# hugocornellier/face_detection_tflite

Hardware: NVIDIA B200
Metric: images/sec BlazeFace detect (pre+infer+NMS) (higher is better)
Workload: dtype f32

## Files before the change

face_detection_tflite_b200/csrc/engine.cu:

```cuda
#include "engine.h"

#include <algorithm>
#include <cstdio>
#include <cstdlib>

namespace fdt {

Engine::~Engine() {
  if (d_blob_) cudaFree(d_blob_);
  for (TailLayerD* p : d_tail_) if (p) cudaFree(p);
  for (TailBlk* p : d_blks_) if (p) cudaFree(p);
}

bool Engine::init(const uint8_t* tflite, size_t len, int fuse_level, std::string* err, bool use_tc) {
  if (!model_.parse(tflite, len, err)) return false;
  if (!plan_.build(model_, fuse_level, err, use_tc)) return false;
  size_t bytes = plan_.blob.size() * sizeof(float) + 64;
  if (cudaMalloc(&d_blob_, bytes) != cudaSuccess) { *err = "cudaMalloc(weights) failed"; return false; }
  cudaMemset(d_blob_, 0, bytes);
  if (cudaMemcpy(d_blob_, plan_.blob.data(), plan_.blob.size() * sizeof(float), cudaMemcpyHostToDevice) != cudaSuccess) {
    *err = "weight upload failed";
    return false;
  }
  d_tail_.assign(plan_.steps.size(), nullptr);
// ... 200 lines not shown
        p.in_floats = st.in_stage_floats;
        if (!launch_block_ws(p, B, ctx.cap, s)) { failed_ = true; fprintf(stderr, "fdt: k_block_ws could not be launched for step '%s'\n", st.name.c_str()); }
        break;
      }
      case kStepTailWs: {
        TailP p;
        TV iv = view(ctx, st.in);
        p.in = iv.p; p.in_istride = iv.istride; p.H = iv.H; p.W = iv.W; p.CinS = iv.Cs;
        p.blob = blob; p.layers = d_tail_[&st - plan_.steps.data()]; p.nlayers = (int)st.tail.size();
        p.nbuf = st.tail_nbuf;
        for (int k = 0; k < kTailMaxBufs; ++k) { p.buf_off[k] = st.tail_buf_off[k]; p.buf_ks[k] = st.tail_buf_ks[k]; }
        p.act_floats = st.tail_act_floats; p.in_bytes = st.tail_in_bytes;
        p.generic = 0;
        for (const TailLayerD& L : st.tail)
          if (L.kind >= 2 || L.act == 2 || L.w_parts != 1 || L.wscale != 1.f || L.rbuf != L.src || (L.kind != 1 && L.o1 >= 0)) p.generic = 1;
        p.blks = nullptr; p.nblks = 0; p.bias_floats = 0; p.in_px = iv.H * iv.W;
        for (int k = 0; k < 2; ++k) { p.rsrc[k] = nullptr; p.rs_istride[k] = 0; p.rs_cs[k] = p.rs_w[k] = p.rs_c[k] = 0; }
        if (st.tail_wide) {
          p.generic = 2;
          p.blks = d_blks_[&st - plan_.steps.data()]; p.nblks = (int)st.tail_blks.size(); p.bias_floats = st.tail_bias_floats;
          for (size_t k = 0; k < st.tail_rsrc.size() && k < 2; ++k) {
            TV rv = view(ctx, st.tail_rsrc[k]);
            p.rsrc[k] = rv.p; p.rs_istride[k] = rv.istride; p.rs_cs[k] = rv.Cs; p.rs_w[k] = rv.W; p.rs_c[k] = rv.C;
          }
        }
        p.last_a_layer = st.tail_last_a; p.wbuf_bytes = st.tail_wbuf; p.wdepth = st.tail_wdepth; p.tbuf_bytes = st.tail_tbuf; p.smem_bytes = st.smem;
        for (int k = 0; k < 4; ++k) { p.outs[k] = nullptr; p.out_istride[k] = 0; p.out_pix[k] = 0; }
        for (size_t k = 0; k < st.tail_outs.size(); ++k) {
          TV ov = view(ctx, st.tail_outs[k]);
          p.outs[k] = ov.p; p.out_istride[k] = ov.istride; p.out_pix[k] = ov.Cs;
        }
        if (!launch_tail_ws(p, B, ctx.cap, s)) { failed_ = true; fprintf(stderr, "fdt: k_tail_ws could not be launched for step '%s'\n", st.name.c_str()); }
        break;
      }
      case kStepFcTc: {
        FcP p;
        TV iv = view(ctx, st.in);
        p.in = iv.p; p.in_istride = iv.istride;
        p.out = out.p; p.out_istride = out.istride;
        p.w = blob + st.w; p.bias = blob + st.bias;
        p.K = st.K; p.K16 = st.K8; p.N = st.Cout; p.w_parts = st.w_parts; p.tile_bytes = st.ts_rec_bytes; p.wscale = (float)st.out_scale;
        if (!launch_fc_tc(p, B, s)) { failed_ = true; fprintf(stderr, "fdt: k_fc_tc could not be launched for step '%s'\n", st.name.c_str()); }
        break;
      }
      case kStepBlockTs: {
        BlockTsP p;
        TV iv = view(ctx, st.in);
        p.in = iv.p; p.in_istride = iv.istride; p.H = iv.H; p.W = iv.W; p.CinS = iv.Cs;
        p.out = out.p; p.out_istride = out.istride; p.OH = out.H; p.OW = out.W; p.CoutS = out.Cs;
        p.rec = blob + st.ts_rec; p.bias = blob + st.ts_bias; p.rec_bytes = st.ts_rec_bytes;
        p.Cin = iv.C; p.K16 = st.ts_k16; p.Npad = st.ts_npad; p.KS = st.ts_ks;
        p.stride = st.dws; p.res = st.ts_res; p.relu = st.ts_relu;
        p.wide = (out.Cs % 8 == 0 && out.istride % 8 == 0 && ((size_t)out.p % 32 == 0)) ? 1 : 0;
        p.ns = st.ts_ns; p.stage_bytes = st.ts_stage_bytes; p.smem_bytes = st.smem;
        {
          const float* hdw = plan_.blob.data() + st.ts_rec + (size_t)st.ts_npad * st.ts_k16 / 2;
          for (int q = 0; q < 16; ++q)
            for (int k = 0; k < 10; ++k)
              for (int c = 0; c < 4; ++c) p.dw[(q * 10 + k) * 4 + c] = 4 * q + c < st.ts_k16 ? hdw[k * st.ts_k16 + 4 * q + c] : 0.f;
        }
        if (!launch_block_ts(p, B, ctx.cap, s)) { failed_ = true; fprintf(stderr, "fdt: k_block_ts could not be launched for step '%s'\n", st.name.c_str()); }
        break;
      }
      case kStepAdd: case kStepAct: case kStepPadC: {
        EltP p;
        p.a = view(ctx, st.in);
        p.b = st.in2 >= 0 ? view(ctx, st.in2) : p.a;
        p.out = out;
        p.alpha = st.alpha >= 0 ? blob + st.alpha : nullptr;
        p.act = st.act;
        if (st.kind == kStepAdd) launch_add(p, B, s);
        else if (st.kind == kStepAct) launch_act(p, B, s);
        else launch_padc(p, B, s);
        break;
      }
      case kStepMaxPool: {
        PoolP p;
        p.in = view(ctx, st.in); p.out = out;
        p.fh = st.fh; p.fw = st.fw; p.sh = st.sh; p.sw = st.sw; p.pt = st.pt; p.pl = st.pl;
        launch_maxpool(p, B, s);
        break;
      }
      case kStepResize: {
        ResizeP p;
        p.in = view(ctx, st.in); p.out = out; p.align_corners = st.align; p.half_pixel = st.half;
        p.has_add = st.in2 >= 0 ? 1 : 0; p.act = st.act;
        p.add = st.in2 >= 0 ? view(ctx, st.in2) : p.in;
        launch_resize_bilinear(p, B, s);
        break;
      }
    }
    ++launches;
  }
  if (evs) cudaEventRecord(evs[launches], s);
  return launches;
}

}
```

face_detection_tflite_b200/csrc/fdt_api.cu:

```cuda
#include <cuda_runtime.h>

#include <algorithm>
#include <cmath>
#include <cstdio>
#include <cstdlib>
#include <cstring>
#include <mutex>
#include <string>
#include <thread>
#include <vector>

#include "../../include/fdt_api.h"
#include "engine.h"
#include "jpeg_host.h"
#include "fdt_math.h"
#include "kernels.h"
#include "tile_walk.h"

using namespace fdt;

static_assert(sizeof(fdt_face) == 160, "fdt_face wire layout (bindings rely on it)");
static_assert(sizeof(fdt_config) == 48, "fdt_config layout");

namespace {
// ... 1533 lines not shown
  std::lock_guard<std::mutex> g(h->mu);
  const int S = (int)h->det.plan().steps.size();
  if (out_launches) *out_launches = S + 2;
  FrameLayout lay;
  const char* msg = nullptr;
  if (!d_frames || n <= 0 || n > h->chunk || width <= 0 || height <= 0 || repeats <= 0 ||
      frame_layout(mat_type, width, height, row_stride, &lay, &msg) != FDT_OK)
    return fail(h, FDT_ERR_BAD_ARG, "bad profile arguments");
  if (!out_ms || capacity < S + 2) return fail(h, FDT_ERR_SIZE_MISMATCH, "out_ms too small");
  cudaSetDevice(h->cfg.device);
  if (!ensure_results(h, n)) return FDT_ERR_CUDA;
  const LbTables* tb = get_tables(h, width, height);
  if (!tb) return fail(h, FDT_ERR_CUDA, "letterbox table upload failed");
  std::vector<cudaEvent_t> ev(S + 3);
  for (auto& e : ev) cudaEventCreate(&e);
  std::vector<double> acc(S + 2, 0.0);
  Slot& sl = h->slots[0];
  cudaStream_t s = sl.stream;
  const int S_w = h->det.in_w(), S_h = h->det.in_h();
  for (int r = 0; r < repeats; ++r) {
    cudaEventRecord(ev[0], s);
    if (lay.yuv) {
      LetterboxYuvP lb;
      fill_letterbox_yuv(lb, tb, lay, d_frames, lay.frame_bytes, false, d_frames + lay.c_off, lay.frame_bytes, false, row_stride,
                         width, height, sl.d_lb, S_w, S_h);
      launch_letterbox_yuv(lb, n, s);
    } else {
      LetterboxP lb;
      fill_letterbox(lb, tb, d_frames, lay.frame_bytes, row_stride, lay.channels, width, height, sl.d_lb, S_w, S_h, false);
      launch_letterbox(lb, n, s);
    }
    h->det.run(sl.det_ctx, sl.d_lb, n, s, ev.data() + 1);
    DecodeP d;
    fill_decode(d, h, sl, tb, width, height);
    d.faces = h->d_faces; d.counts = h->d_counts;
    launch_decode_nms(d, n, s);
    cudaEventRecord(ev[S + 2], s);
    if (!cuda_ok(h, cudaStreamSynchronize(s), "profile")) { for (auto& e : ev) cudaEventDestroy(e); return FDT_ERR_CUDA; }
    for (int i = 0; i < S + 2; ++i) {
      float ms = 0;
      cudaEventElapsedTime(&ms, ev[i], ev[i + 1]);
      acc[i] += ms;
    }
  }
  for (int i = 0; i < S + 2; ++i) out_ms[i] = (float)(acc[i] / repeats);
  for (auto& e : ev) cudaEventDestroy(e);
  return FDT_OK;
}

static const char* kKernelNames[] = {"k_normalize", "k_naive_conv", "k_gemm_conv", "k_dwpw", "k_add", "k_act", "k_padc", "k_maxpool",
                                     "k_resize_bilinear", "k_stem", "k_block_ws", "k_stem_ws", "k_tail_ws", "k_fc_tc", "k_block_ts"};

static void step_info(const Plan& p, const PStep& st, int in_w, int in_h, std::string* kname, std::string* tname, double* macs, double* bytes) {
  *kname = kKernelNames[st.kind]; *tname = st.name; *macs = st.macs;
  const PTensor& o = p.tensors[st.out];
  double b = (double)o.H * o.W * o.C * 4;
  if (st.out2 >= 0) { const PTensor& o2 = p.tensors[st.out2]; b += (double)o2.H * o2.W * o2.C * 4; }
  if (st.in_u8) b += (double)in_w * in_h * 4;
  else if (st.in >= 0) { const PTensor& i = p.tensors[st.in]; b += (double)i.H * i.W * i.C * 4; }
  if (st.in2 >= 0 && st.in2 != st.in) { const PTensor& r = p.tensors[st.in2]; b += (double)r.H * r.W * r.C * 4; }
  for (int extra : st.extra_out) { const PTensor& e = p.tensors[extra]; b += (double)e.H * e.W * e.C * 4; }
  *bytes = b;
}

int32_t fdt_get_step_info(fdt_handle* h, int32_t launch, char* kernel, char* tensor, int32_t str_cap, double* macs_per_image,
                          double* bytes_per_image) {
  if (!h || !h->ready) return fail(h, FDT_ERR_NOT_READY, "detector is not initialised");
  h = primary(h);
  const Plan& p = h->det.plan();
  const int S = (int)p.steps.size();
  if (launch < 0 || launch > S + 1) return fail(h, FDT_ERR_BAD_ARG, "launch index out of range");
  std::string kname, tname;
  double macs = 0, bytes = 0;
  if (launch == 0) {
    kname = "k_letterbox"; tname = "letterboxed_u8";
    bytes = 0;
  } else if (launch == S + 1) {
    kname = "k_decode_nms"; tname = "faces";
    bytes = (double)h->num_anchors * 17 * 4;
  } else {
    step_info(p, p.steps[launch - 1], h->det.in_w(), h->det.in_h(), &kname, &tname, &macs, &bytes);
  }
  if (kernel && str_cap > 0) { std::snprintf(kernel, str_cap, "%s", kname.c_str()); }
  if (tensor && str_cap > 0) { std::snprintf(tensor, str_cap, "%s", tname.c_str()); }
  if (macs_per_image) *macs_per_image = macs;
  if (bytes_per_image) *bytes_per_image = bytes;
  return FDT_OK;
}

int32_t fdt_profile_net(fdt_handle* h, int32_t which, int32_t n, int32_t repeats, float* out_ms, int32_t capacity, int32_t* out_steps) {
  if (!h || !h->ready) return fail(h, FDT_ERR_NOT_READY, "detector is not initialised");
  h = primary(h);
  std::lock_guard<std::mutex> g(h->mu);
  if (which != 1 && which != 2) return fail(h, FDT_ERR_BAD_ARG, "which: 1 mesh, 2 iris");
  if ((which == 1 && !h->has_mesh) || (which == 2 && !h->has_iris)) return fail(h, FDT_ERR_NOT_READY, "model not loaded");
  const Engine& e = which == 1 ? h->mesh : h->iris;
  const int S = (int)e.plan().steps.size();
  if (out_steps) *out_steps = S;
  const int have = which == 1 ? h->last_mesh_faces : 2 * h->last_iris_faces;
  if (n <= 0 || n > have) n = have;
  if (out_steps) out_steps[0] = S;
  if (n <= 0 || repeats <= 0) return fail(h, FDT_ERR_BAD_ARG, "the last call left no crops in the stage buffers");
  if (!out_ms || capacity < S) return fail(h, FDT_ERR_SIZE_MISMATCH, "out_ms too small");
  cudaSetDevice(h->cfg.device);
  Slot& sl = h->slots[which == 1 ? h->last_mesh_slot : h->last_iris_slot];
  cudaStream_t s = sl.stream;
  std::vector<cudaEvent_t> ev(S + 1);
// ... 124 lines not shown
```

face_detection_tflite_b200/csrc/kernels.h:

```cpp
#pragma once
#include <cuda_runtime.h>
#include <algorithm>
#include <cstdint>

#include "../../include/fdt_api.h"
#include "tail_layer.h"

namespace fdt {

enum { kActNone = 0, kActRelu = 1, kActPrelu = 2 };

struct FastDiv {
  unsigned mul = 0, shr = 0, d = 1;
  FastDiv() {}
  explicit FastDiv(int div) {
    d = div < 1 ? 1u : (unsigned)div;
    unsigned l = 0;
    while ((1ull << l) < d) ++l;
    shr = l;
    mul = (unsigned)(((1ull << 32) * ((1ull << l) - d)) / d + 1);
  }
#ifdef __CUDACC__
  __device__ __forceinline__ int div(int n) const { return (int)((__umulhi(mul, (unsigned)n) + (unsigned)n) >> shr); }
  __device__ __forceinline__ void divmod(int n, int& q, int& r) const { q = div(n); r = n - q * (int)d; }
// ... 104 lines not shown
  size_t smem_bytes;
};
void launch_dwpw(const DwPwP& p, int B, cudaStream_t s, int max_ctas);

struct DwPwTcP {
  const float* in; long long in_istride; int H, W, Cin, CinS;
  int has_dw, s, dpt, dpl, OH, OW;
  const float* dww;
  const float* dwb;
  int K8, KS;
  float* out; long long out_istride; int Cout, CoutS, vec_store;
  const float* wB;
  const float* bias; const float* alpha;
  int act, Npad, tmem_cols, a_rows, RS;
  int in_floats, n_chunks, n_items;
  int nr, KSr, res_stage_floats;
  int deint, plane_floats, PW;
  int w_parts;
  int nbuf;
  int ns, na, nd, nt;
  int no, KSo, out_stage_floats;
  float* out2; long long out2_istride; int Cs2, c1, c2;
  long long* trace;
  const float* res; long long res_istride; int res_H, res_W, res_C, res_Cs, res_pool, res_mode, res_lim;
  int TH, TW, G, IH, IW, tilesX, tilesY;
  FastDiv fd_Q8, fd_IW, fd_IH, fd_TW, fd_thw, fd_tpg, fd_tilesX, fd_nstrips, fd_nslots;
  size_t smem_bytes;
};
bool launch_block_ws(const DwPwTcP& p, int B, int cap, cudaStream_t s);

struct StemWsP {
  const uint8_t* in8;
  int H, W, OH, OW, kw, pt, pl;
  float* out; long long out_istride; int Cout, CoutS, vec_store;
  const float* wB;
  const float* bias; const float* alpha;
  int act, Npad, K8, tmem_cols, w_parts;
  float out_scale;
  size_t smem_bytes;
};
bool launch_stem_ws(const StemWsP& p, int B, int cap, cudaStream_t s);

struct BlockTsP {
  const float* in; long long in_istride; int H, W, CinS;
  float* out; long long out_istride; int OH, OW, CoutS;
  const float* rec;
  const float* bias;
  int rec_bytes;
  int Cin, K16, Npad, KS;
  int stride;
  int res;
  int relu, wide;
  int ns, stage_bytes;
  size_t smem_bytes;
  alignas(16) float dw[10 * 64];
};
size_t ts_smem_bytes(int rec_bytes, int Npad, int ns, int stage_bytes);
bool launch_block_ts(const BlockTsP& p, int B, int cap, cudaStream_t s);

struct TailP {
  const float* in; long long in_istride; int H, W, CinS;
  const float* blob;
  const TailLayerD* layers;
  int nlayers;
  int nbuf;
  int buf_off[kTailMaxBufs];
  int buf_ks[kTailMaxBufs];
  int act_floats;
  int in_bytes;
  int last_a_layer;
  int wbuf_bytes, wdepth;
  int tbuf_bytes;
  int generic;
  const TailBlk* blks; int nblks; int bias_floats; int in_px;
  const float* rsrc[2]; long long rs_istride[2]; int rs_cs[2], rs_w[2], rs_c[2];
  float* outs[4]; long long out_istride[4]; int out_pix[4];
  size_t smem_bytes;
};
size_t tail_smem_bytes(int act_floats, int wbuf_bytes, int wdepth, int tbuf_bytes);
size_t wide_smem_bytes(int act_floats, int wbuf_bytes, int wdepth, int tbuf_bytes, int bias_floats);
bool launch_tail_ws(const TailP& p, int B, int cap, cudaStream_t s);

struct FcP {
  const float* in; long long in_istride;
  float* out; long long out_istride;
  const float* w;
  const float* bias;
  int K, K16, N, w_parts, tile_bytes;
  float wscale;
};
bool launch_fc_tc(const FcP& p, int B, cudaStream_t s);

struct JpegIdctP {
  const int16_t* coef;
  const uint16_t* q;
  int bw, bh;
  uint8_t* plane; int pitch;
};
struct JpegColorP {
  const uint8_t* py; const uint8_t* pcb; const uint8_t* pcr;
  int pitch_y, pitch_c;
  int W, H, ncomp;
  int cdw, cdh, hs, vs;
  int orientation;
  uint8_t* out; int out_w;
};
// ... 59 lines not shown
```

face_detection_tflite_b200/csrc/kernels_ts.cu:

```cuda
#include <cuda.h>
#include <cuda_fp16.h>

#include <algorithm>
#include <cstdio>
#include <map>
#include <mutex>
#include <tuple>
#include <type_traits>

#include "kernels.h"
#include "tile_walk.h"

namespace fdt {
namespace {

constexpr int kC = 12;
constexpr int kThreads = (kC + 2) * 32;
constexpr uint32_t kLBO = 128;

__device__ __forceinline__ uint32_t smem_u32(const void* p) { return (uint32_t)__cvta_generic_to_shared(p); }
__device__ __forceinline__ void mbar_init(uint32_t bar, uint32_t count) { asm volatile("mbarrier.init.shared::cta.b64 [%0], %1;" ::"r"(bar), "r"(count)); }
__device__ __forceinline__ void mbar_arrive(uint32_t bar) { asm volatile("mbarrier.arrive.shared::cta.b64 _, [%0];" ::"r"(bar) : "memory"); }
__device__ __forceinline__ void mbar_expect_tx(uint32_t bar, uint32_t bytes) {
  asm volatile("mbarrier.arrive.expect_tx.shared::cta.b64 _, [%0], %1;" ::"r"(bar), "r"(bytes) : "memory");
// ... 245 lines not shown
        if (lane == 0) mbar_arrive(in_empty + 8u * (uint32_t)stage);
      }
      at_prev = at; stage_prev = stage;
      tile_advance(at, step, tiles_x, tiles_y);
      if (++stage == NS) { stage = 0; in_phase ^= 1u; }
    }
    if (n_my > 0) epilogue(n_my - 1, stage_prev, at_prev.b, at_prev.ty, at_prev.tx);
  } else if (warp == kC) {
    if (lane == 0) {
      const TileStep step = tile_step((int)gridDim.x, tpi, tiles_x);
      TileAt at = tile_at((int)blockIdx.x, tpi, tiles_x);
      int stage = 0;
      uint32_t empty_phase = 1;
      for (int i = 0; i < n_my; ++i) {
        const int b = at.b, ty = at.ty, tx = at.tx;
        if (i >= NS) mbar_wait_idle(in_empty + 8u * (uint32_t)stage, empty_phase);
        const uint32_t bar = in_full + 8u * (uint32_t)stage;
        mbar_expect_tx(bar, (uint32_t)((S == 1 ? 18 * 18 : 2 * 17 * 17) * KS) * 4u);
        const int ix0 = S == 1 ? tx * TW - 1 : tx * TW * 2, iy0 = S == 1 ? ty * TH - 1 : ty * TH * 2;
        asm volatile("cp.async.bulk.tensor.4d.shared::cluster.global.mbarrier::complete_tx::bytes [%0], [%1, {%2, %3, %4, %5}], [%6];"
                     ::"r"(ring_a + (uint32_t)stage * stage_b), "l"(&tmap), "r"(0), "r"(ix0), "r"(iy0), "r"(b), "r"(bar) : "memory");
        if (S == 2)
          asm volatile("cp.async.bulk.tensor.4d.shared::cluster.global.mbarrier::complete_tx::bytes [%0], [%1, {%2, %3, %4, %5}], [%6];"
                       ::"r"(ring_a + (uint32_t)stage * stage_b + plane_b), "l"(&tmap), "r"(0), "r"(ix0 + 1), "r"(iy0), "r"(b), "r"(bar) : "memory");
        tile_advance(at, step, tiles_x, tiles_y);
        if (++stage == NS) { stage = 0; empty_phase ^= 1u; }
      }
    }
    __syncwarp();
  } else {
    if (lane == 0) {
      const uint32_t idesc = (1u << 4) | ((uint32_t)(p.Npad >> 3) << 17) | ((128u >> 4) << 24);
      const uint32_t sbo = (uint32_t)(p.K16 >> 3) * 128u;
      const uint32_t b_hi = ((sbo >> 4) & 0x3FFFu) | (1u << 14);
      const uint32_t b_lo0 = ((smem_u32(sRec) & 0x3FFFFu) >> 4) | ((kLBO >> 4) << 16);
      const int ksteps = p.K16 >> 4;
      for (int i = 0; i < n_my; ++i) {
        const int slot = i & 1;
        mbar_wait_idle(a_full + 8u * (uint32_t)slot, (uint32_t)((i >> 1) & 1));
        asm volatile("tcgen05.fence::after_thread_sync;" ::: "memory");
#pragma unroll
        for (int t = 0; t < NT; ++t) {
          const uint32_t dcol = tmem_base + col_d(slot, t), acol = tmem_base + col_a(slot, t);
          uint32_t acc = 0u;
#pragma unroll 1
          for (int part = 0; part < 2; ++part)
#pragma unroll 1
            for (int ks = 0; ks < ksteps; ++ks) {
              mma_ts_f16(dcol, acol + 32u * (uint32_t)part + 8u * (uint32_t)ks, b_lo0 + 16u * (uint32_t)ks, b_hi, idesc, acc);
              acc = 1u;
            }
        }
        asm volatile("tcgen05.commit.cta_group::1.mbarrier::arrive::one.shared::cluster.b64 [%0];" ::"r"(d_full + 8u * (uint32_t)slot) : "memory");
      }
    }
    __syncwarp();
  }
  asm volatile("tcgen05.fence::before_thread_sync;" ::: "memory");
  __syncthreads();
  if (warp == kC + 1) {
    asm volatile("tcgen05.fence::after_thread_sync;" ::: "memory");
    asm volatile("tcgen05.dealloc.cta_group::1.sync.aligned.b32 %0, %1;" ::"r"(tmem_base), "r"(512u));
  }
}

typedef CUresult (*EncodeTiledFn)(CUtensorMap*, CUtensorMapDataType, cuuint32_t, void*, const cuuint64_t*, const cuuint64_t*,
                                  const cuuint32_t*, const cuuint32_t*, CUtensorMapInterleave, CUtensorMapSwizzle,
                                  CUtensorMapL2promotion, CUtensorMapFloatOOBfill);

EncodeTiledFn encode_fn() {
  static EncodeTiledFn fn = [] {
    void* f = nullptr;
    cudaDriverEntryPointQueryResult q;
    if (cudaGetDriverEntryPoint("cuTensorMapEncodeTiled", &f, cudaEnableDefault, &q) != cudaSuccess || q != cudaDriverEntryPointSuccess) f = nullptr;
    return (EncodeTiledFn)f;
  }();
  return fn;
}

bool ts_tensor_map(const BlockTsP& p, int cap, CUtensorMap* out) {
  typedef std::tuple<const void*, int, int, int, int, int, int, long long> Key;
  static std::mutex mu;
  static std::map<Key, CUtensorMap> cache;
  Key key(p.in, cap, p.H, p.W, p.CinS, p.KS, p.stride, p.in_istride);
  std::lock_guard<std::mutex> g(mu);
  auto it = cache.find(key);
  if (it != cache.end()) { *out = it->second; return true; }
  EncodeTiledFn enc = encode_fn();
  if (!enc) return false;
  cuuint64_t gdim[4] = {(cuuint64_t)p.CinS, (cuuint64_t)p.W, (cuuint64_t)p.H, (cuuint64_t)cap};
  cuuint64_t gstr[3] = {(cuuint64_t)p.CinS * 4, (cuuint64_t)p.W * p.CinS * 4, (cuuint64_t)p.in_istride * 4};
  cuuint32_t box[4] = {(cuuint32_t)p.KS, p.stride == 1 ? 18u : 33u, p.stride == 1 ? 18u : 17u, 1u};
  cuuint32_t estr[4] = {1, p.stride == 1 ? 1u : 2u, 1, 1};
  CUtensorMap tm;
  CUresult r = enc(&tm, CU_TENSOR_MAP_DATA_TYPE_FLOAT32, 4, const_cast<float*>(p.in), gdim, gstr, box, estr,
                   CU_TENSOR_MAP_INTERLEAVE_NONE, CU_TENSOR_MAP_SWIZZLE_NONE, CU_TENSOR_MAP_L2_PROMOTION_L2_128B,
                   CU_TENSOR_MAP_FLOAT_OOB_FILL_NONE);
  if (r != CUDA_SUCCESS) return false;
  if (cache.size() > 256) cache.clear();
  cache[key] = tm;
  *out = tm;
  return true;
}

template <int S, int KSC>
bool launch_ts(const CUtensorMap& tm, const BlockTsP& p, int B, cudaStream_t s) {
  static std::mutex mu;
  static std::map<int, size_t> cur;
  int dev = 0, sms = 148;
  cudaGetDevice(&dev);
  cudaDeviceGetAttribute(&sms, cudaDevAttrMultiProcessorCount, dev);
  {
    std::lock_guard<std::mutex> g(mu);
    size_t& c = cur[dev];
    if (p.smem_bytes > c) {
      if (cudaFuncSetAttribute(k_block_ts<S, KSC>, cudaFuncAttributeMaxDynamicSharedMemorySize, (int)p.smem_bytes) != cudaSuccess) return false;
      c = p.smem_bytes;
    }
  }
  const int ntiles = B * (p.OW / 16) * (p.OH / (S == 1 ? 16 : 8));
  const int grid = std::max(1, std::min(ntiles, sms));
  k_block_ts<S, KSC><<<grid, kThreads, p.smem_bytes, s>>>(tm, p, B);
  return true;
}

}

size_t ts_smem_bytes(int rec_bytes, int Npad, int ns, int stage_bytes) {
  return (size_t)rec_bytes + (size_t)Npad * 4 + 32 * 8 + 128 + (size_t)ns * stage_bytes + 128;
}

bool launch_block_ts(const BlockTsP& p, int B, int cap, cudaStream_t s) {
  if (B <= 0) return true;
  CUtensorMap tm;
  if (!ts_tensor_map(p, cap, &tm)) return false;
  if (p.stride == 1) {
    switch (p.KS) {
      case 28: return launch_ts<1, 28>(tm, p, B, s);
      case 36: return launch_ts<1, 36>(tm, p, B, s);
      case 44: return launch_ts<1, 44>(tm, p, B, s);
      case 52: return launch_ts<1, 52>(tm, p, B, s);
      default: return launch_ts<1, 0>(tm, p, B, s);
    }
  }
  switch (p.KS) {
    case 28: return launch_ts<2, 28>(tm, p, B, s);
    case 36: return launch_ts<2, 36>(tm, p, B, s);
    case 44: return launch_ts<2, 44>(tm, p, B, s);
    case 52: return launch_ts<2, 52>(tm, p, B, s);
    default: return launch_ts<2, 0>(tm, p, B, s);
  }
}

}
```

face_detection_tflite_b200/csrc/plan.cpp:

```cpp
#include "plan.h"

#include <algorithm>
#include <cmath>
#include <cstdio>
#include <cstdlib>
#include <cstring>
#include <cstdint>

namespace fdt {
namespace {

constexpr size_t kSmemLimit = 200 * 1024;
constexpr int kActNone = 0, kActRelu = 1, kActPrelu = 2;

inline int ru(int v, int m) { return (v + m - 1) / m * m; }
inline int smem_stride(int KP) { return KP + (((KP / 4) % 2 == 0) ? 4 : 0); }

void same_pad(int in, int k, int s, int* before) {
  int out = (in + s - 1) / s;
  int total = (out - 1) * s + k - in;
  if (total < 0) total = 0;
  *before = total / 2;
}

// ... 376 lines not shown
    }
    if (st.has_dw) {
      const TfOp& dw = m.ops[absorbed[0]];
      std::vector<float> dwv, dbv;
      if (!m.const_f32(dw.in[1], &dwv) || !m.const_f32(dw.in[2], &dbv)) return fail("depthwise weights are not constant");
      const int kp = tc ? fs.K8 : st.KP;
      std::vector<float> dk((size_t)9 * kp, 0.f);
      for (int t = 0; t < 9; ++t)
        for (int c = 0; c < Cin; ++c) dk[(size_t)t * kp + c] = dwv[(size_t)t * Cin + c];
      F->st.dww = push(dk, dk.size());
      F->st.dwb = push(dbv, kp);
    }
    F->st.macs = (double)OH * OW * ((double)Cin * st.Cout + (st.has_dw ? 9.0 * Cin : 0.0));
    if (tc && F->st.kind == kStepBlockWs) plan_ts(&F->st, st_in, OH, OW, alpha_tf >= 0);
    return true;
  }

  void plan_ts(PStep* st, const TfTensor& in, int OH, int OW, bool prelu) {
    static const int want = [] { const char* e = std::getenv("FDT_TS"); return e ? std::atoi(e) : 1; }();
    if (!want || !st->has_dw || st->c2 > 0 || st->w_parts != 1 || prelu) return;
    if (st->act != kActRelu && st->act != kActNone) return;
    const int Cin = in.dim(3), K16 = ru(Cin, 16), Npad = ru(st->Cout, 16);
    if (K16 > 64 || Npad > 64) return;
    if (st->dws == 1 ? (OH % 16 || OW % 16 || st->dpt != 1 || st->dpl != 1)
                     : (OH % 8 || OW % 16 || st->dpt != 0 || st->dpl != 0 || in.dim(1) != 2 * OH || in.dim(2) != 2 * OW)) return;
    int res = 0;
    if (st->res_mode != 0) {
      if (st->res_mode != 1) return;
      res = st->res_pool ? 2 : 1;
      if ((res == 2) != (st->dws == 2)) return;
    }
    const size_t SBO8 = (size_t)(st->K8 / 4) * 128, SBO16 = (size_t)(K16 / 8) * 128;
    std::vector<uint16_t> wh((size_t)Npad * K16, 0);
    for (int n = 0; n < st->Cout; ++n)
      for (int k = 0; k < Cin; ++k) {
        const float v = P.blob[(size_t)st->w + ((size_t)(n >> 3) * SBO8 + (size_t)(k >> 2) * 128 + (size_t)(n & 7) * 16 + (size_t)(k & 3) * 4) / 4];
        const uint16_t hbits = f32_to_f16(v);
        if (f16_to_f32(hbits) != v) return;
        wh[((size_t)(n >> 3) * SBO16 + (size_t)(k >> 3) * 128 + (size_t)(n & 7) * 16 + (size_t)(k & 7) * 2) / 2] = hbits;
      }
    std::vector<float> rec(wh.size() / 2 + (size_t)10 * K16, 0.f);
    std::memcpy(rec.data(), wh.data(), wh.size() * 2);
    float* dw = rec.data() + wh.size() / 2;
    for (int k = 0; k < 9; ++k)
      for (int c = 0; c < Cin; ++c) dw[(size_t)k * K16 + c] = P.blob[(size_t)st->dww + (size_t)k * st->K8 + c];
    for (int c = 0; c < Cin; ++c) dw[(size_t)9 * K16 + c] = P.blob[(size_t)st->dwb + c];
    std::vector<float> bias((size_t)Npad, 0.f);
    for (int n = 0; n < st->Cout; ++n) bias[n] = P.blob[(size_t)st->bias + n];
    const int KS = odd_quads(ru(Cin, 4));
    const int stage_bytes = st->dws == 1 ? (18 * 18 * KS * 4 + 127) / 128 * 128 : 2 * ((17 * 17 * KS * 4 + 127) / 128 * 128);
    const size_t head = rec.size() * 4 + (size_t)Npad * 4 + 32 * 8 + 256;
    int ns = (int)(((size_t)220 * 1024 - head) / stage_bytes);
    if (ns < 2) return;
    if (ns > 4) ns = 4;
    st->ts_rec = push(rec, rec.size());
    st->ts_bias = push(bias, bias.size());
    st->ts_rec_bytes = (int)(rec.size() * 4);
    st->ts_k16 = K16; st->ts_npad = Npad; st->ts_ks = KS; st->ts_ns = ns; st->ts_stage_bytes = stage_bytes;
    st->ts_res = res; st->ts_relu = st->act == kActRelu ? 1 : 0;
    st->TH = st->dws == 1 ? 16 : 8; st->TW = 16; st->G = 1;
    st->smem = head + (size_t)ns * stage_bytes;
    st->kind = kStepBlockTs;
  }

  static void split_w(float v, int parts, float* hi, float* lo) {
    if (parts == 1) { *hi = v; return; }
    uint32_t u;
    std::memcpy(&u, &v, 4);
    u &= 0xFFFFE000u;
    float h;
    std::memcpy(&h, &u, 4);
    *hi = h;
    *lo = v - h;
  }

  static bool tf32_exact(const std::vector<float>& w) {
    for (float v : w) {
      uint32_t u;
      std::memcpy(&u, &v, 4);
      if (u & 0x1FFFu) return false;
    }
    return true;
  }

  bool plan_tc(PStep* st, int Cin, int OH, int OW, int w_parts) {
    PStep s = *st;
    s.w_parts = w_parts;
    s.K8 = ru(Cin, 8);
    s.Npad = ru(s.Cout, 16);
    if (s.Npad > 128 || s.K8 > 256) return false;
    s.KS = s.K8 + (((s.K8 / 4) % 2 == 0) ? 4 : 0);
    s.tmem_cols = 32;
    while (s.tmem_cols < s.Npad) s.tmem_cols *= 2;
    for (int Pn = 128; Pn >= 32; Pn /= 2) {
      const size_t cap = (size_t)220 * 1024;
      s.TM = 1; s.NPG = Pn;
      int bestTH = 0, bestTW = 0, bestG = 1;
      double best = -1;
      if (OH * OW <= Pn && OW <= 30) {
        bestTH = OH; bestTW = OW; bestG = std::min(63, Pn / (OH * OW));
      } else {
        for (int TW = std::min(std::min(OW, Pn), 30); TW >= 1; --TW) {
          int TH = std::min(std::min(OH, Pn / TW), 30);
          if (TH < 1) continue;
          double tiles = (double)((OH + TH - 1) / TH) * ((OW + TW - 1) / TW);
          double util = (double)OH * OW / (tiles * Pn);
          double halo = (double)((TH - 1) * s.dws + 3) * ((TW - 1) * s.dws + 3) / ((double)TH * TW * s.dws * s.dws);
          double score = util / (s.has_dw ? halo : 1.0);
          if (score > best + 1e-9) { best = score; bestTH = TH; bestTW = TW; }
        }
      }
      s.TH = bestTH; s.TW = bestTW; s.G = bestG;
// ... 1060 lines not shown
      if (fuse == 1) {
        for (Block& b : blocks) {
          if (b.free_after < x.def_step && b.size >= need) {
            x.arena_off = b.off;
            b.free_after = x.last_use;
            placed = true;
            break;
          }
        }
      }
      if (!placed) {
        x.arena_off = top;
        blocks.push_back({top, need, x.last_use});
        top += need;
      }
    }
    P.arena_per_image = top;
    return true;
  }
};

}

bool Plan::build(const TfModel& m, int fuse, std::string* err, bool use_tc) {
  *this = Plan();
  fuse_level = fuse;
  Builder b(m, *this, fuse);
  b.use_tc = use_tc;
  bool ok = b.run();
  if (!ok && err) *err = b.err;
  return ok;
}

std::string Plan::describe() const {
  static const char* kn[] = {"normalize", "naive_conv", "gemm_conv", "dwpw", "add", "act", "padc", "maxpool", "resize", "stem", "block_ws", "stem_ws", "tail_ws", "fc_tc", "block_ts"};
  std::string s;
  char buf[512];
  double macs = 0;
  for (size_t i = 0; i < steps.size(); ++i) {
    const PStep& st = steps[i];
    const PTensor& o = tensors[st.out];
    macs += st.macs;
    snprintf(buf, sizeof buf,
             "%3zu %-10s in=%d res=%d%s/m%d out=%d[%dx%dx%d Cs%d %s] act=%d dw=%d/s%d K=%d NC=%dx%d TM=%d NPG=%d tile=%dx%dx%d RS=%d nd=%d ns=%d na=%d no=%d smem=%zu  %s\n",
             i, kn[st.kind], st.in >= 0 ? tensors[st.in].tf : -1, st.in2 >= 0 ? tensors[st.in2].tf : -1,
             st.res_pool ? "(pool)" : "", st.res_mode, o.tf, o.H, o.W, o.C, o.Cs, o.root >= 0 ? "view" : "arena", st.act,
             (int)st.has_dw, st.dws, st.K, st.NC, st.nchunks, st.TM, st.NPG, st.TH, st.TW, st.G, st.RS, st.nd, st.ns, st.na, st.no, st.smem, st.name.c_str());
    s += buf;
    if (st.kind == kStepBlockWs && (st.nr > 0 || st.deint)) {
      snprintf(buf, sizeof buf, "      k_block_ws: residual ring %d x %d B (record %d floats)%s\n", st.nr, st.res_stage_floats * 4, st.KSr,
               st.deint ? ", stride 2 on even / odd column planes" : "");
      s += buf;
    }
    if (st.tail_wide) {
      snprintf(buf, sizeof buf, "      k_chain_wide: %zu W blocks (ring %d x %d B), act %d floats, %zu HBM residual tensor(s)\n", st.tail_blks.size(), st.tail_wdepth, st.tail_wbuf,
               st.tail_act_floats, st.tail_rsrc.size());
      s += buf;
    }
    for (size_t l = 0; l < st.tail.size(); ++l) {
      const TailLayerD& L = st.tail[l];
      static const char* lk[] = {"block", "heads", "pw", "dot"};
      snprintf(buf, sizeof buf, "      tail %2zu %s buf %d->%d %dx%d->%dx%d s%d C %d->%d K16=%d Npad=%d res=%d(buf %d) act=%d wparts=%d out=%d rec=%dB taps=%dB\n", l, lk[L.kind & 3],
               L.src, L.dst, L.IH, L.IW, L.OH, L.OW, L.stride, L.Cin, L.Cout, L.K16, L.Npad, L.res, L.rbuf, L.act, L.w_parts, L.o1, L.rec_bytes, L.tap_bytes);
      s += buf;
      if (st.tail_wide && L.kind != 3) {
        s.pop_back();
        snprintf(buf, sizeof buf, " wide: groups=%d blocks/group=%d Kchunks=%d blk0=%d\n", L.ng & 0xff, L.ng >> 8, L.nk, L.blk0);
        s += buf;
      }
    }
  }
  snprintf(buf, sizeof buf, "steps=%zu  MACs/image=%.3fM  arena/image=%.1f KB  weights=%.1f KB\n", steps.size(),
           macs / 1e6, arena_per_image * 4.0 / 1024, blob.size() * 4.0 / 1024);
  s += buf;
  return s;
}

}
```

face_detection_tflite_b200/csrc/plan.h:

```cpp
#pragma once
#include <map>
#include <string>
#include <vector>

#include "tail_layer.h"
#include "tflite_model.h"

namespace fdt {

struct PTensor {
  int tf = -1;
  int H = 1, W = 1, C = 1, Cs = 1;
  long long istride = 0;
  int root = -1;
  long long view_off = 0;
  long long arena_off = -1;
  int def_step = -1, last_use = -1;
  bool materialized = false;
  bool is_input = false;
};

enum StepKind { kStepNormalize, kStepNaiveConv, kStepGemmConv, kStepDwPw, kStepAdd, kStepAct, kStepPadC,
                kStepMaxPool, kStepResize, kStepStem, kStepBlockWs, kStepStemWs, kStepTailWs, kStepFcTc, kStepBlockTs };

struct PStep {
  StepKind kind = kStepAct;
  std::string name;
  int in = -1, in2 = -1, out = -1;
  int kh = 1, kw = 1, sh = 1, sw = 1, pt = 0, pl = 0, act = 0, depthwise = 0;
  bool in_u8 = false;
  bool has_dw = false;
  int dws = 1, dpt = 0, dpl = 0, res_pool = 0, res_mode = 0;
  long long w = -1, bias = -1, alpha = -1, dww = -1, dwb = -1;
  int K = 0, KP = 0, KS = 0, Cout = 0, CoutP = 0, NC = 0, nchunks = 0, NPG = 0, TM = 0;
  int TH = 0, TW = 0, G = 1, IH = 0, IW = 0, tilesX = 1, tilesY = 1;
  size_t smem = 0;
  int K8 = 0, Npad = 0, a_rows = 0, RS = 1, tmem_cols = 0, w_parts = 1, nbuf = 1;
  double out_scale = 1.0;
  int ns = 0, na = 0, nd = 8, nt = 2, in_stage_floats = 0;
  int no = 0, KSo = 0, out_stage_floats = 0;
  int nr = 0, KSr = 0, res_stage_floats = 0;
  int deint = 0, plane_floats = 0, PW = 0;
  int out2 = -1, c1 = 0, c2 = 0;
  int fh = 1, fw = 1, align = 0, half = 0;
  std::vector<int> extra_out;
  long long ts_rec = -1, ts_bias = -1;
  int ts_rec_bytes = 0, ts_k16 = 0, ts_npad = 0, ts_ks = 0, ts_ns = 0, ts_stage_bytes = 0, ts_res = 0, ts_relu = 0;
  std::vector<TailLayerD> tail;
  std::vector<int> tail_outs;
  int tail_nbuf = 0, tail_buf_off[kTailMaxBufs] = {0}, tail_buf_ks[kTailMaxBufs] = {0}, tail_buf_px[kTailMaxBufs] = {0};
  std::vector<TailBlk> tail_blks;
  std::vector<int> tail_rsrc;
  int tail_wide = 0, tail_bias_floats = 0;
  int tail_act_floats = 0, tail_in_bytes = 0, tail_last_a = 0, tail_wbuf = 0, tail_wdepth = 2, tail_tbuf = 0;
  double macs = 0;
};

struct Plan {
  std::vector<PTensor> tensors;
  std::vector<PStep> steps;
  std::vector<float> blob;
  std::map<int, int> tf2pt;
  int input = -1, in_h = 0, in_w = 0;
  std::vector<int> outputs;
  std::vector<long long> out_elems;
  long long arena_per_image = 0;
  int fuse_level = 1;

  bool build(const TfModel& m, int fuse_level, std::string* err, bool use_tc = true);
  std::string describe() const;
};

}
```

face_detection_tflite_b200/csrc/tile_walk.h:

```cpp
#pragma once

#ifdef __CUDACC__
#define FDT_HD __host__ __device__ __forceinline__
#else
#define FDT_HD inline
#endif

namespace fdt {

struct TileAt { int b, ty, tx; };
struct TileStep { int b, ty, tx; };

FDT_HD TileAt tile_at(int tile, int tpi, int tiles_x) {
  TileAt a;
  a.b = tile / tpi;
  const int r = tile - a.b * tpi;
  a.ty = r / tiles_x; a.tx = r - a.ty * tiles_x;
  return a;
}
FDT_HD TileStep tile_step(int stride, int tpi, int tiles_x) {
  const TileAt a = tile_at(stride, tpi, tiles_x);
  TileStep s; s.b = a.b; s.ty = a.ty; s.tx = a.tx;
  return s;
}
FDT_HD void tile_advance(TileAt& a, const TileStep& s, int tiles_x, int tiles_y) {
  a.tx += s.tx; a.ty += s.ty; a.b += s.b;
  if (a.tx >= tiles_x) { a.tx -= tiles_x; ++a.ty; }
  if (a.ty >= tiles_y) { a.ty -= tiles_y; ++a.b; }
}

}
```

Before: 775,600.

## Add warp-group-per-tile variant of tensor-core block kernel with deeper ring

Adds k_block_ts_wg, in which three warp groups each own a whole tile and rotate through TMEM column sets, so depthwise compute, MMA and epilogue of different tiles overlap. The MMA warp commits per group, and the input ring grows to up to 6 stages for eligible layers (K16<=32, Npad<=32, Cout%8==0). It is enabled by default through the FDT_TS_WG env var, and the launcher refuses unsupported shapes. In exchange it brings more template instantiations, more shared memory for the ring, and new synchronisation complexity.

After: 793,500, median of 6. 2.3% higher.

```diff
diff --git a/face_detection_tflite_b200/csrc/engine.cu b/face_detection_tflite_b200/csrc/engine.cu
--- a/face_detection_tflite_b200/csrc/engine.cu
+++ b/face_detection_tflite_b200/csrc/engine.cu
@@ -276,7 +276,7 @@
         p.Cin = iv.C; p.K16 = st.ts_k16; p.Npad = st.ts_npad; p.KS = st.ts_ks;
         p.stride = st.dws; p.res = st.ts_res; p.relu = st.ts_relu;
         p.wide = (out.Cs % 8 == 0 && out.istride % 8 == 0 && ((size_t)out.p % 32 == 0)) ? 1 : 0;
-        p.ns = st.ts_ns; p.stage_bytes = st.ts_stage_bytes; p.smem_bytes = st.smem;
+        p.ns = st.ts_ns; p.stage_bytes = st.ts_stage_bytes; p.wg = st.ts_wg; p.smem_bytes = st.smem;
         {
           const float* hdw = plan_.blob.data() + st.ts_rec + (size_t)st.ts_npad * st.ts_k16 / 2;
           for (int q = 0; q < 16; ++q)
diff --git a/face_detection_tflite_b200/csrc/fdt_api.cu b/face_detection_tflite_b200/csrc/fdt_api.cu
--- a/face_detection_tflite_b200/csrc/fdt_api.cu
+++ b/face_detection_tflite_b200/csrc/fdt_api.cu
@@ -1609,7 +1609,7 @@
                                      "k_resize_bilinear", "k_stem", "k_block_ws", "k_stem_ws", "k_tail_ws", "k_fc_tc", "k_block_ts"};
 
 static void step_info(const Plan& p, const PStep& st, int in_w, int in_h, std::string* kname, std::string* tname, double* macs, double* bytes) {
-  *kname = kKernelNames[st.kind]; *tname = st.name; *macs = st.macs;
+  *kname = st.kind == kStepBlockTs && st.ts_wg ? "k_block_ts_wg" : kKernelNames[st.kind]; *tname = st.name; *macs = st.macs;
   const PTensor& o = p.tensors[st.out];
   double b = (double)o.H * o.W * o.C * 4;
   if (st.out2 >= 0) { const PTensor& o2 = p.tensors[st.out2]; b += (double)o2.H * o2.W * o2.C * 4; }
diff --git a/face_detection_tflite_b200/csrc/kernels.h b/face_detection_tflite_b200/csrc/kernels.h
--- a/face_detection_tflite_b200/csrc/kernels.h
+++ b/face_detection_tflite_b200/csrc/kernels.h
@@ -180,6 +180,7 @@
   int res;
   int relu, wide;
   int ns, stage_bytes;
+  int wg;
   size_t smem_bytes;
   alignas(16) float dw[10 * 64];
 };
diff --git a/face_detection_tflite_b200/csrc/kernels_ts.cu b/face_detection_tflite_b200/csrc/kernels_ts.cu
--- a/face_detection_tflite_b200/csrc/kernels_ts.cu
+++ b/face_detection_tflite_b200/csrc/kernels_ts.cu
@@ -321,6 +321,250 @@
             }
         }
         asm volatile("tcgen05.commit.cta_group::1.mbarrier::arrive::one.shared::cluster.b64 [%0];" ::"r"(d_full + 8u * (uint32_t)slot) : "memory");
+      }
+    }
+    __syncwarp();
+  }
+  asm volatile("tcgen05.fence::before_thread_sync;" ::: "memory");
+  __syncthreads();
+  if (warp == kC + 1) {
+    asm volatile("tcgen05.fence::after_thread_sync;" ::: "memory");
+    asm volatile("tcgen05.dealloc.cta_group::1.sync.aligned.b32 %0, %1;" ::"r"(tmem_base), "r"(512u));
+  }
+}
+
+__device__ __forceinline__ uint32_t wg_col_d(int g, int t) { return (uint32_t)(g * 128 + t * 64); }
+__device__ __forceinline__ uint32_t wg_col_a(int g, int t) { return (uint32_t)(g * 128 + t * 64 + 32); }
+constexpr uint32_t kWgLoOff = 16;
+
+template <int S, int NQ>
+__global__ void __launch_bounds__(kThreads, 1) k_block_ts_wg(const __grid_constant__ CUtensorMap tmap, const __grid_constant__ BlockTsP p, int B) {
+  extern __shared__ __align__(128) unsigned char smem_raw[];
+  __shared__ uint32_t tmem_base_s;
+  constexpr int NT = S == 1 ? 2 : 1;
+  constexpr int TH = S == 1 ? 16 : 8, TW = 16;
+  constexpr int IW = S == 1 ? 18 : 17;
+  constexpr int KS = 4 * (NQ | 1);
+  constexpr int K16 = (4 * NQ + 15) / 16 * 16, NQP = K16 / 4;
+  constexpr int ks_q = KS / 4;
+  constexpr uint32_t ks_b = KS * 4u, row_b = IW * ks_b;
+  constexpr uint32_t plane_b = (17u * 17u * ks_b + 127u) & ~127u;
+  constexpr uint32_t col2_b[3] = {0u, plane_b, ks_b};
+  const int tid = threadIdx.x, warp = tid >> 5, lane = tid & 31;
+  float* sRec = reinterpret_cast<float*>(smem_raw);
+  float* sBias = sRec + (p.rec_bytes >> 2);
+  uint64_t* bars = reinterpret_cast<uint64_t*>(sBias + p.Npad);
+  unsigned char* ring = reinterpret_cast<unsigned char*>((reinterpret_cast<uintptr_t>(bars + 32) + 127) & ~(uintptr_t)127);
+  const uint32_t bar0 = smem_u32(bars);
+  const uint32_t in_full = bar0, in_empty = bar0 + 64u, a_full = bar0 + 128u, d_full = bar0 + 152u;
+  const int NS = p.ns;
+  const int tiles_x = p.OW / TW, tiles_y = p.OH / TH, tpi = tiles_x * tiles_y;
+  const int ntiles = B * tpi;
+  const int n_my = (int)blockIdx.x < ntiles ? (ntiles - 1 - (int)blockIdx.x) / (int)gridDim.x + 1 : 0;
+
+  for (int i = tid; i < (p.rec_bytes >> 4); i += kThreads) reinterpret_cast<uint4*>(sRec)[i] = reinterpret_cast<const uint4*>(p.rec)[i];
+  for (int i = tid; i < p.Npad; i += kThreads) sBias[i] = p.bias[i];
+  if (tid < 2) bars[24 + tid] = 0ull;
+  if (tid == 0) {
+    for (int i = 0; i < NS; ++i) { mbar_init(in_full + 8u * i, 1); mbar_init(in_empty + 8u * i, 4); }
+    for (int i = 0; i < 3; ++i) { mbar_init(a_full + 8u * i, 4); mbar_init(d_full + 8u * i, 1); }
+    asm volatile("fence.mbarrier_init.release.cluster;" ::: "memory");
+    asm volatile("prefetch.tensormap [%0];" ::"l"(&tmap) : "memory");
+  }
+  if (warp == kC + 1) {
+    asm volatile("tcgen05.alloc.cta_group::1.sync.aligned.shared::cta.b32 [%0], %1;" ::"r"(smem_u32(&tmem_base_s)), "r"(512u));
+    asm volatile("tcgen05.relinquish_alloc_permit.cta_group::1.sync.aligned;" ::);
+  }
+  asm volatile("fence.proxy.async.shared::cta;" ::: "memory");
+  asm volatile("tcgen05.fence::before_thread_sync;" ::: "memory");
+  __syncthreads();
+  asm volatile("tcgen05.fence::after_thread_sync;" ::: "memory");
+  const uint32_t tmem_base = tmem_base_s;
+  const uint32_t ring_a = smem_u32(ring);
+  const uint32_t stage_b = (uint32_t)p.stage_bytes;
+
+  if (warp < kC) {
+    const int lq = warp & 3, g = warp >> 2;
+    const int L = lq * 32 + lane;
+    const int yy = L >> 4, x = L & 15;
+    const uint32_t tm_lane = tmem_base + ((uint32_t)(lq * 32) << 16);
+    const uint32_t win = (uint32_t)((2 * yy) * IW + x) * ks_b;
+    const uint32_t bias_a = smem_u32(sBias), zero_a = bar0 + 192u;
+    const int couts = p.CoutS, nc8 = (couts + 7) >> 3;
+    const uint32_t acol0 = tm_lane + wg_col_a(g, 0), acol1 = tm_lane + wg_col_a(g, 1);
+    const uint32_t dcol0 = tm_lane + wg_col_d(g, 0);
+    const float4 zero4 = make_float4(0.f, 0.f, 0.f, 0.f);
+#pragma unroll
+    for (int q = NQ; q < NQP; ++q) {
+      split_store_tmem(acol0 + 2u * q, kWgLoOff, zero4);
+      if (S == 1) split_store_tmem(acol1 + 2u * q, kWgLoOff, zero4);
+    }
+    if (NQP > NQ) asm volatile("tcgen05.wait::st.sync.aligned;" ::: "memory");
+    const int n_g = n_my > g ? (n_my - 1 - g) / 3 + 1 : 0;
+    const TileStep step = tile_step(3 * (int)gridDim.x, tpi, tiles_x);
+    TileAt at = tile_at((int)blockIdx.x + g * (int)gridDim.x, tpi, tiles_x);
+    RingAt rs = ring_at(g, NS);
+    for (int k = 0; k < n_g; ++k) {
+      mbar_wait(in_full + 8u * (uint32_t)rs.stage, rs.phase);
+      const uint32_t st_a = ring_a + (uint32_t)rs.stage * stage_b + win;
+#pragma unroll
+      for (int q = 0; q < NQ; ++q) {
+        const float4* cw = reinterpret_cast<const float4*>(p.dw) + 10 * q;
+        float4 w[9];
+#pragma unroll
+        for (int j = 0; j < 9; ++j) w[j] = cw[j];
+        const float4 bias = cw[9];
+        const uint32_t pa = st_a + 16u * q;
+        float4 a0 = bias, a1;
+        if (S == 1) {
+          float4 v[3];
+#pragma unroll
+          for (int c = 0; c < 3; ++c) v[c] = lds4(pa + c * ks_b);
+#pragma unroll
+          for (int c = 0; c < 3; ++c) fma4(a0, v[c], w[c]);
+#pragma unroll
+          for (int c = 0; c < 3; ++c) v[c] = lds4(pa + row_b + c * ks_b);
+          a1 = bias;
+#pragma unroll
+          for (int c = 0; c < 3; ++c) { fma4(a0, v[c], w[3 + c]); fma4(a1, v[c], w[c]); }
+#pragma unroll
+          for (int c = 0; c < 3; ++c) v[c] = lds4(pa + 2u * row_b + c * ks_b);
+#pragma unroll
+          for (int c = 0; c < 3; ++c) { fma4(a0, v[c], w[6 + c]); fma4(a1, v[c], w[3 + c]); }
+#pragma unroll
+          for (int c = 0; c < 3; ++c) v[c] = lds4(pa + 3u * row_b + c * ks_b);
+#pragma unroll
+          for (int c = 0; c < 3; ++c) fma4(a1, v[c], w[6 + c]);
+          split_store_tmem(acol1 + 2u * q, kWgLoOff, a1);
+        } else {
+#pragma unroll
+          for (int j = 0; j < 9; ++j) fma4(a0, lds4(pa + (uint32_t)(j / 3) * row_b + col2_b[j % 3]), w[j]);
+        }
+        split_store_tmem(acol0 + 2u * q, kWgLoOff, a0);
+      }
+      asm volatile("tcgen05.wait::st.sync.aligned;" ::: "memory");
+      asm volatile("tcgen05.fence::before_thread_sync;" ::: "memory");
+      __syncwarp();
+      if (lane == 0) mbar_arrive(a_full + 8u * (uint32_t)g);
+      float4 rvp[8];
+      if (S == 2) {
+#pragma unroll
+        for (int cq = 0; cq < 8; ++cq) {
+          rvp[cq] = zero4;
+          if (p.res == 2 && cq < ks_q && cq < 2 * nc8)
+            rvp[cq] = max4(max4(lds4(st_a + 16u * cq), lds4(st_a + plane_b + 16u * cq)),
+                           max4(lds4(st_a + row_b + 16u * cq), lds4(st_a + row_b + plane_b + 16u * cq)));
+        }
+        __syncwarp();
+        if (lane == 0) mbar_arrive(in_empty + 8u * (uint32_t)rs.stage);
+      }
+      mbar_wait(d_full + 8u * (uint32_t)g, (uint32_t)(k & 1));
+      asm volatile("tcgen05.fence::after_thread_sync;" ::: "memory");
+      float* const orow0 = p.out + (size_t)at.b * p.out_istride + (uint32_t)(((at.ty * TH + (S == 1 ? 2 * yy : yy)) * p.OW + at.tx * TW + x) * couts);
+      const uint32_t orow_step = (uint32_t)(p.OW * couts);
+#pragma unroll
+      for (int t = 0; t < NT; ++t) {
+        float* orow = orow0 + (t ? orow_step : 0u);
+        const uint32_t res_a = st_a + (uint32_t)(t + 1) * row_b + ks_b;
+        const uint32_t dcol = dcol0 + (uint32_t)t * 64u;
+        auto unit = [&](auto c8c, auto ngc) {
+          constexpr int C8 = decltype(c8c)::value, NG = decltype(ngc)::value;
+          uint32_t u[8 * NG];
+          if (NG == 2)
+            asm volatile(
+                "tcgen05.ld.sync.aligned.32x32b.x16.b32 {%0, %1, %2, %3, %4, %5, %6, %7, %8, %9, %10, %11, %12, %13, %14, %15}, [%16];"
+                : "=r"(u[0]), "=r"(u[1]), "=r"(u[2]), "=r"(u[3]), "=r"(u[4]), "=r"(u[5]), "=r"(u[6]), "=r"(u[7]),
+                  "=r"(u[8 * (NG - 1)]), "=r"(u[8 * (NG - 1) + 1]), "=r"(u[8 * (NG - 1) + 2]), "=r"(u[8 * (NG - 1) + 3]),
+                  "=r"(u[8 * (NG - 1) + 4]), "=r"(u[8 * (NG - 1) + 5]), "=r"(u[8 * (NG - 1) + 6]), "=r"(u[8 * (NG - 1) + 7])
+                : "r"(dcol + 8u * C8));
+          else
+            asm volatile("tcgen05.ld.sync.aligned.32x32b.x8.b32 {%0, %1, %2, %3, %4, %5, %6, %7}, [%8];"
+                         : "=r"(u[0]), "=r"(u[1]), "=r"(u[2]), "=r"(u[3]), "=r"(u[4]), "=r"(u[5]), "=r"(u[6]), "=r"(u[7])
+                         : "r"(dcol + 8u * C8));
+          float4 bv[2 * NG], rv[2 * NG];
+#pragma unroll
+          for (int j = 0; j < 2 * NG; ++j) {
+            const int cq = 2 * C8 + j;
+            bv[j] = lds4(bias_a + 16u * cq);
+            if (S == 2) rv[j] = rvp[cq];
+            else rv[j] = lds4(p.res == 1 && cq < ks_q ? res_a + 16u * cq : zero_a);
+          }
+          asm volatile("tcgen05.wait::ld.sync.aligned;" ::: "memory");
+          float4 v[2 * NG];
+#pragma unroll
+          for (int j = 0; j < 2 * NG; ++j) {
+            v[j] = make_float4(__uint_as_float(u[4 * j]) + bv[j].x + rv[j].x, __uint_as_float(u[4 * j + 1]) + bv[j].y + rv[j].y,
+                               __uint_as_float(u[4 * j + 2]) + bv[j].z + rv[j].z, __uint_as_float(u[4 * j + 3]) + bv[j].w + rv[j].w);
+            if (p.relu) v[j] = max4(v[j], zero4);
+          }
+#pragma unroll
+          for (int kk = 0; kk < NG; ++kk) {
+            const int c = 8 * (C8 + kk);
+            if (c + 8 <= couts) {
+              if (p.wide) stg8(orow + c, v[2 * kk], v[2 * kk + 1]);
+              else { *reinterpret_cast<float4*>(orow + c) = v[2 * kk]; *reinterpret_cast<float4*>(orow + c + 4) = v[2 * kk + 1]; }
+            } else if (c + 4 <= couts) {
+              *reinterpret_cast<float4*>(orow + c) = v[2 * kk];
+            }
+          }
+        };
+        if (nc8 >= 2) unit(std::integral_constant<int, 0>(), std::integral_constant<int, 2>());
+        if (nc8 == 1) unit(std::integral_constant<int, 0>(), std::integral_constant<int, 1>());
+        if (nc8 == 3) unit(std::integral_constant<int, 2>(), std::integral_constant<int, 1>());
+        if (nc8 == 4) unit(std::integral_constant<int, 2>(), std::integral_constant<int, 2>());
+      }
+      asm volatile("tcgen05.fence::before_thread_sync;" ::: "memory");
+      __syncwarp();
+      if (S == 1 && lane == 0) mbar_arrive(in_empty + 8u * (uint32_t)rs.stage);
+      tile_advance(at, step, tiles_x, tiles_y);
+      ring_advance(rs, 3, NS);
+    }
+  } else if (warp == kC) {
+    if (lane == 0) {
+      const TileStep step = tile_step((int)gridDim.x, tpi, tiles_x);
+      TileAt at = tile_at((int)blockIdx.x, tpi, tiles_x);
+      int stage = 0;
+      uint32_t empty_phase = 1;
+      for (int i = 0; i < n_my; ++i) {
+        if (i >= NS) mbar_wait_idle(in_empty + 8u * (uint32_t)stage, empty_phase);
+        const uint32_t bar = in_full + 8u * (uint32_t)stage;
+        mbar_expect_tx(bar, (uint32_t)((S == 1 ? 18 * 18 : 2 * 17 * 17) * KS) * 4u);
+        const int ix0 = S == 1 ? at.tx * TW - 1 : at.tx * TW * 2, iy0 = S == 1 ? at.ty * TH - 1 : at.ty * TH * 2;
+        asm volatile("cp.async.bulk.tensor.4d.shared::cluster.global.mbarrier::complete_tx::bytes [%0], [%1, {%2, %3, %4, %5}], [%6];"
+                     ::"r"(ring_a + (uint32_t)stage * stage_b), "l"(&tmap), "r"(0), "r"(ix0), "r"(iy0), "r"(at.b), "r"(bar) : "memory");
+        if (S == 2)
+          asm volatile("cp.async.bulk.tensor.4d.shared::cluster.global.mbarrier::complete_tx::bytes [%0], [%1, {%2, %3, %4, %5}], [%6];"
+                       ::"r"(ring_a + (uint32_t)stage * stage_b + plane_b), "l"(&tmap), "r"(0), "r"(ix0 + 1), "r"(iy0), "r"(at.b), "r"(bar) : "memory");
+        tile_advance(at, step, tiles_x, tiles_y);
+        if (++stage == NS) { stage = 0; empty_phase ^= 1u; }
+      }
+    }
+    __syncwarp();
+  } else {
+    if (lane == 0) {
+      const uint32_t idesc = (1u << 4) | ((uint32_t)(p.Npad >> 3) << 17) | ((128u >> 4) << 24);
+      constexpr uint32_t sbo = (uint32_t)(K16 >> 3) * 128u;
+      const uint32_t b_hi = ((sbo >> 4) & 0x3FFFu) | (1u << 14);
+      const uint32_t b_lo0 = ((smem_u32(sRec) & 0x3FFFFu) >> 4) | ((kLBO >> 4) << 16);
+      int g = 0;
+      uint32_t par = 0;
+      for (int i = 0; i < n_my; ++i) {
+        mbar_wait_idle(a_full + 8u * (uint32_t)g, par);
+        asm volatile("tcgen05.fence::after_thread_sync;" ::: "memory");
+#pragma unroll
+        for (int t = 0; t < NT; ++t) {
+          const uint32_t dcol = tmem_base + wg_col_d(g, t), acol = tmem_base + wg_col_a(g, t);
+          uint32_t acc = 0u;
+#pragma unroll
+          for (int part = 0; part < 2; ++part)
+#pragma unroll
+            for (int ks = 0; ks < K16 / 16; ++ks) {
+              mma_ts_f16(dcol, acol + kWgLoOff * part + 8u * ks, b_lo0 + 16u * ks, b_hi, idesc, acc);
+              acc = 1u;
+            }
+        }
+        asm volatile("tcgen05.commit.cta_group::1.mbarrier::arrive::one.shared::cluster.b64 [%0];" ::"r"(d_full + 8u * (uint32_t)g) : "memory");
+        if (++g == 3) { g = 0; par ^= 1u; }
       }
     }
     __syncwarp();
@@ -372,25 +616,47 @@
   return true;
 }
 
-template <int S, int KSC>
-bool launch_ts(const CUtensorMap& tm, const BlockTsP& p, int B, cudaStream_t s) {
+template <typename Kernel>
+bool launch_kernel_ts(Kernel kern, int S, const CUtensorMap& tm, const BlockTsP& p, int B, cudaStream_t s) {
   static std::mutex mu;
-  static std::map<int, size_t> cur;
+  static std::map<std::pair<const void*, int>, size_t> cur;
   int dev = 0, sms = 148;
   cudaGetDevice(&dev);
   cudaDeviceGetAttribute(&sms, cudaDevAttrMultiProcessorCount, dev);
   {
     std::lock_guard<std::mutex> g(mu);
-    size_t& c = cur[dev];
+    size_t& c = cur[std::make_pair((const void*)kern, dev)];
     if (p.smem_bytes > c) {
-      if (cudaFuncSetAttribute(k_block_ts<S, KSC>, cudaFuncAttributeMaxDynamicSharedMemorySize, (int)p.smem_bytes) != cudaSuccess) return false;
+      if (cudaFuncSetAttribute(kern, cudaFuncAttributeMaxDynamicSharedMemorySize, (int)p.smem_bytes) != cudaSuccess) return false;
       c = p.smem_bytes;
     }
   }
   const int ntiles = B * (p.OW / 16) * (p.OH / (S == 1 ? 16 : 8));
   const int grid = std::max(1, std::min(ntiles, sms));
-  k_block_ts<S, KSC><<<grid, kThreads, p.smem_bytes, s>>>(tm, p, B);
+  kern<<<grid, kThreads, p.smem_bytes, s>>>(tm, p, B);
   return true;
+}
+template <int S, int KSC>
+bool launch_ts(const CUtensorMap& tm, const BlockTsP& p, int B, cudaStream_t s) { return launch_kernel_ts(k_block_ts<S, KSC>, S, tm, p, B, s); }
+
+template <int S, int NQ>
+bool launch_ts_wg_nq(const CUtensorMap& tm, const BlockTsP& p, int B, cudaStream_t s) {
+  if (p.KS != 4 * (NQ | 1) || p.K16 != (4 * NQ + 15) / 16 * 16 || p.Npad > 32 || p.ns < 3) return false;
+  return launch_kernel_ts(k_block_ts_wg<S, NQ>, S, tm, p, B, s);
+}
+template <int S>
+bool launch_ts_wg(const CUtensorMap& tm, const BlockTsP& p, int B, cudaStream_t s) {
+  switch ((p.Cin + 3) >> 2) {
+    case 1: return launch_ts_wg_nq<S, 1>(tm, p, B, s);
+    case 2: return launch_ts_wg_nq<S, 2>(tm, p, B, s);
+    case 3: return launch_ts_wg_nq<S, 3>(tm, p, B, s);
+    case 4: return launch_ts_wg_nq<S, 4>(tm, p, B, s);
+    case 5: return launch_ts_wg_nq<S, 5>(tm, p, B, s);
+    case 6: return launch_ts_wg_nq<S, 6>(tm, p, B, s);
+    case 7: return launch_ts_wg_nq<S, 7>(tm, p, B, s);
+    case 8: return launch_ts_wg_nq<S, 8>(tm, p, B, s);
+    default: return false;
+  }
 }
 
 }
@@ -403,6 +669,7 @@
   if (B <= 0) return true;
   CUtensorMap tm;
   if (!ts_tensor_map(p, cap, &tm)) return false;
+  if (p.wg) return p.stride == 1 ? launch_ts_wg<1>(tm, p, B, s) : launch_ts_wg<2>(tm, p, B, s);
   if (p.stride == 1) {
     switch (p.KS) {
       case 28: return launch_ts<1, 28>(tm, p, B, s);
diff --git a/face_detection_tflite_b200/csrc/plan.cpp b/face_detection_tflite_b200/csrc/plan.cpp
--- a/face_detection_tflite_b200/csrc/plan.cpp
+++ b/face_detection_tflite_b200/csrc/plan.cpp
@@ -452,12 +452,14 @@
     const size_t head = rec.size() * 4 + (size_t)Npad * 4 + 32 * 8 + 256;
     int ns = (int)(((size_t)220 * 1024 - head) / stage_bytes);
     if (ns < 2) return;
-    if (ns > 4) ns = 4;
+    static const int want_wg = [] { const char* e = std::getenv("FDT_TS_WG"); return e ? std::atoi(e) : 1; }();
+    const int wg = want_wg && K16 <= 32 && Npad <= 32 && st->Cout % 8 == 0 && ns >= 3 ? 1 : 0;
+    if (ns > (wg ? 6 : 4)) ns = wg ? 6 : 4;
     st->ts_rec = push(rec, rec.size());
     st->ts_bias = push(bias, bias.size());
     st->ts_rec_bytes = (int)(rec.size() * 4);
     st->ts_k16 = K16; st->ts_npad = Npad; st->ts_ks = KS; st->ts_ns = ns; st->ts_stage_bytes = stage_bytes;
-    st->ts_res = res; st->ts_relu = st->act == kActRelu ? 1 : 0;
+    st->ts_res = res; st->ts_relu = st->act == kActRelu ? 1 : 0; st->ts_wg = wg;
     st->TH = st->dws == 1 ? 16 : 8; st->TW = 16; st->G = 1;
     st->smem = head + (size_t)ns * stage_bytes;
     st->kind = kStepBlockTs;
@@ -1624,6 +1626,11 @@
                st.deint ? ", stride 2 on even / odd column planes" : "");
       s += buf;
     }
+    if (st.kind == kStepBlockTs) {
+      snprintf(buf, sizeof buf, "      k_block_ts%s: K16=%d Npad=%d KS=%d ring %d x %d B\n", st.ts_wg ? "_wg (one tile per warp group)" : "",
+               st.ts_k16, st.ts_npad, st.ts_ks, st.ts_ns, st.ts_stage_bytes);
+      s += buf;
+    }
     if (st.tail_wide) {
       snprintf(buf, sizeof buf, "      k_chain_wide: %zu W blocks (ring %d x %d B), act %d floats, %zu HBM residual tensor(s)\n", st.tail_blks.size(), st.tail_wdepth, st.tail_wbuf,
                st.tail_act_floats, st.tail_rsrc.size());
diff --git a/face_detection_tflite_b200/csrc/plan.h b/face_detection_tflite_b200/csrc/plan.h
--- a/face_detection_tflite_b200/csrc/plan.h
+++ b/face_detection_tflite_b200/csrc/plan.h
@@ -46,6 +46,7 @@
   std::vector<int> extra_out;
   long long ts_rec = -1, ts_bias = -1;
   int ts_rec_bytes = 0, ts_k16 = 0, ts_npad = 0, ts_ks = 0, ts_ns = 0, ts_stage_bytes = 0, ts_res = 0, ts_relu = 0;
+  int ts_wg = 0;
   std::vector<TailLayerD> tail;
   std::vector<int> tail_outs;
   int tail_nbuf = 0, tail_buf_off[kTailMaxBufs] = {0}, tail_buf_ks[kTailMaxBufs] = {0}, tail_buf_px[kTailMaxBufs] = {0};
diff --git a/face_detection_tflite_b200/csrc/tile_walk.h b/face_detection_tflite_b200/csrc/tile_walk.h
--- a/face_detection_tflite_b200/csrc/tile_walk.h
+++ b/face_detection_tflite_b200/csrc/tile_walk.h
@@ -29,4 +29,11 @@
   if (a.ty >= tiles_y) { a.ty -= tiles_y; ++a.b; }
 }
 
+struct RingAt { int stage; unsigned phase; };
+FDT_HD RingAt ring_at(int first, int ns) { RingAt r; r.stage = first % ns; r.phase = (unsigned)(first / ns) & 1u; return r; }
+FDT_HD void ring_advance(RingAt& r, int step, int ns) {
+  r.stage += step;
+  if (r.stage >= ns) { r.stage -= ns; r.phase ^= 1u; }
 }
+
+}
```
